# rdspring1/lightning-thunder

Hardware: AMD Instinct MI355X
Metric: tokens/sec/GPU Llama-2-7B pretrain (LitGPT) + speedup vs eager at 1/2/4/8 MI355X (higher is better)
Workload: dtype bf16; 1 GPU; model=Llama-2-7b-hf, global_batch=1, micro_batch=1, seq_len=4096, parallelism=single, mode=thunder, optimizer=AdamW

## Files before the change

lightning_thunder_amd/ops/csrc/attention_bwd.hip:

```cpp
#include "attention.h"

using namespace lta;
using namespace lta::attn;

namespace {

constexpr int kThreads = 256;
typedef __attribute__((address_space(3))) void lds_void;
typedef float f32x4v __attribute__((ext_vector_type(4)));

template <int D> struct BCfg {
  static constexpr int BN = D > 128 ? 32 : 64;
  static constexpr int NKT = BN / 32;
  static constexpr int RSTR = D + 8;
  static constexpr int TSTR = D + 32;
  static constexpr int CH = D / 8;
  static constexpr int KS = D / 16;
  static constexpr int DT = D / 32;
};

struct RowStrides {
  int64_t b, h, t;
};

// ... 126 lines not shown
  using C = BCfg<D>;
  using F = typename Frag<T>::type;
  constexpr int BUF = 2 * kQT * C::RSTR + 2 * kQT * C::TSTR;
  __shared__ __attribute__((aligned(16))) short smem[2 * BUF];
  __shared__ float s_lse[2][kQT], s_delta[2][kQT];
  __shared__ __attribute__((aligned(16))) unsigned s_qterm[2][DROP ? kQT : 4];

  const int n_kb = (Sk + kKB - 1) / kKB;
  (void)n_kb;
  const int kb = (int)blockIdx.y;
  const int nsplit = SPLIT ? ex.hsplit : 1;
  const int bh = SPLIT ? (int)blockIdx.x / nsplit : (int)blockIdx.x;
  const int hs = SPLIT ? (int)blockIdx.x - bh * nsplit : 0;
  const int b = bh / Hkv, hk = bh % Hkv;
  const int group = Hq / Hkv;
  const int gsz = group / nsplit;
  const int hbase = hk * group + hs * gsz;
  const int tid = threadIdx.x, lane = tid & 63;
  const int wave = __builtin_amdgcn_readfirstlane(tid >> 6);
  const int r = lane & 31, h = lane >> 5, g = lane >> 4, l16 = lane & 15;
  const int kw = kb * kKB + wave * 32;
  const int key = kw + r;
  const T* Kb = K + b * ex.sx.kb + hk * ex.sx.kh;
  const T* Vb = V + b * ex.sx.vb + hk * ex.sx.vh;

  F kf[C::KS], vf[C::KS];
  {
    const int krow = min(key, Sk - 1);
#pragma unroll
    for (int s = 0; s < C::KS; ++s) {
      kf[s] = load_frag<F>(Kb + (int64_t)krow * ex.sx.kt + 16 * s + 8 * h);
      vf[s] = load_frag<F>(Vb + (int64_t)krow * ex.sx.vt + 16 * s + 8 * h);
    }
  }
  f32x16 dkacc[C::DT], dvacc[C::DT];
#pragma unroll
  for (int dt = 0; dt < C::DT; ++dt)
#pragma unroll
    for (int i = 0; i < 16; ++i) {
      dkacc[dt][i] = 0.f;
      dvacc[dt][i] = 0.f;
    }

  const int n_qt = (Tq + kQT - 1) / kQT;
  const int qt_begin = CAUSAL ? min((kb * kKB) / kQT, n_qt) : 0;
  const int nq = n_qt - qt_begin;
  const int total = gsz * nq;
  constexpr int NCH = kQT * C::CH, LOADS = (NCH + kThreads - 1) / kThreads;

  uint4 pq[LOADS], po[LOADS];
  float plse = 0.f, pdel = 0.f;
  auto issue = [&](int it) {
    const int hq = hbase + it / nq;
    const int qbase = (qt_begin + it % nq) * kQT;
    const T* Qb = Q + b * ex.sx.qb + hq * ex.sx.qh;
    const T* dOb = dO + b * sdo.b + hq * sdo.h;
#pragma unroll
    for (int c = 0; c < LOADS; ++c) {
      const int id = c * kThreads + tid;
      if (NCH % kThreads != 0 && id >= NCH) break;
      const int row = id / C::CH, ch = id % C::CH;
      const int qc = min(qbase + row, Tq - 1);
      pq[c] = *reinterpret_cast<const uint4*>(Qb + (int64_t)qc * ex.sx.qt + ch * 8);
      po[c] = *reinterpret_cast<const uint4*>(dOb + qc * sdo.t + ch * 8);
    }
    if (tid < kQT) {
      const int qc = min(qbase + tid, Tq - 1);
      plse = LSE[((int64_t)b * Hq + hq) * Tq + qc];
      pdel = DELTA[((int64_t)b * Hq + hq) * Tq + qc];
    }
  };
  auto stash = [&](int it, int buf) {
    const int qbase = (qt_begin + it % nq) * kQT;
    short* Qr = smem + buf * BUF;
    short* dOr = Qr + kQT * C::RSTR;
    short* Qt = dOr + kQT * C::RSTR;
    short* dOt = Qt + kQT * C::TSTR;
#pragma unroll
    for (int c = 0; c < LOADS; ++c) {
      const int id = c * kThreads + tid;
      if (NCH % kThreads != 0 && id >= NCH) break;
      const int row = id / C::CH, ch = id % C::CH;
      uint4 xq = pq[c], xo = po[c];
      if (qbase + row >= Tq) {
        xq = make_uint4(0, 0, 0, 0);
        xo = make_uint4(0, 0, 0, 0);
      }
      *reinterpret_cast<uint4*>(Qr + row * C::RSTR + ch * 8) = xq;
      *reinterpret_cast<uint4*>(dOr + row * C::RSTR + ch * 8) = xo;
      *reinterpret_cast<uint4*>(Qt + row * C::TSTR + ch * 8) = xq;
      *reinterpret_cast<uint4*>(dOt + row * C::TSTR + ch * 8) = xo;
    }
    if (tid < kQT) {
      const bool ok = qbase + tid < Tq && !(MASK && plse == -INFINITY);
      s_lse[buf][tid] = ok ? plse * 1.44269504088896340736f : INFINITY;
      s_delta[buf][tid] = ok ? pdel : 0.f;
      if constexpr (DROP) s_qterm[buf][tid] = rng_q(rng_head(ex, b * Hq + hbase + it / nq), qbase + tid);
    }
  };

  if (total > 0) {
    issue(0);
    stash(0, 0);
  }
  __syncthreads();
  for (int it = 0; it < total; ++it) {
    const int buf = it & 1;
    const bool more = it + 1 < total;
    if (more) issue(it + 1);
    const int qbase = (qt_begin + it % nq) * kQT;
    const short* Qr = smem + buf * BUF;
    const short* dOr = Qr + kQT * C::RSTR;
    const __attribute__((address_space(3))) short* Qt3 =
        (const __attribute__((address_space(3))) short*)(dOr + kQT * C::RSTR);
    const __attribute__((address_space(3))) short* dOt3 = Qt3 + kQT * C::TSTR;
    const float* sl = s_lse[buf];
    const float* sd = s_delta[buf];

    f32x16 sacc, pacc;
#pragma unroll
    for (int i = 0; i < 16; ++i) {
      sacc[i] = 0.f;
      pacc[i] = 0.f;
    }
#pragma unroll
    for (int s = 0; s < C::KS; ++s) {
      const F qa = load_frag<F>(Qr + r * C::RSTR + 16 * s + 8 * h);
      const F oa = load_frag<F>(dOr + r * C::RSTR + 16 * s + 8 * h);
      sacc = mfma(qa, kf[s], sacc);
      pacc = mfma(oa, vf[s], pacc);
    }
    [[maybe_unused]] const int hq_it = hbase + it / nq;
    [[maybe_unused]] unsigned kterm = 0;
    if constexpr (DROP) kterm = rng_k(key);
#pragma unroll
    for (int i = 0; i < 16; ++i) {
      const int qr = acc_row(i, h);
      const int qq = qbase + qr;
      float sv = sacc[i] * scale_log2;
      if constexpr (MASK)
        sv += ex.mask[b * ex.mb + hq_it * ex.mh + (int64_t)min(qq, Tq - 1) * ex.mq + min(key, Sk - 1)] *
              1.44269504088896340736f;
      float p = __builtin_amdgcn_exp2f(sv - sl[qr]);
      p = (key >= Sk || qq >= Tq || (CAUSAL && key > qq)) ? 0.f : p;
      float dp = pacc[i];
      float pd = p;
      if constexpr (DROP) {
        const uint4 qv = rng_tab4(s_qterm[buf], i >> 2, h);
        const unsigned qw4[4] = {qv.x, qv.y, qv.z, qv.w};
        const bool keep = rng_keep(ex, qw4[i & 3], kterm);
        pd = keep ? p * ex.keep_scale : 0.f;
        dp = keep ? dp * ex.keep_scale : 0.f;
      }
      sacc[i] = pd;
      pacc[i] = p * (dp - sd[qr]);
      if constexpr (MGRAD) {
        if (key < Sk && qq < Tq) ex.dmask[(((int64_t)b * Hq + hq_it) * Tq + qq) * Sk + key] = pacc[i];
      }
    }
    F pf0, pf1, df0, df1;
    pack_frag(pf0, sacc, 0);
    pack_frag(pf1, sacc, 1);
    pack_frag(df0, pacc, 0);
    pack_frag(df1, pacc, 1);
#pragma unroll
    for (int dt = 0; dt < C::DT; ++dt) {
      const int col0 = dt * 32 + 16 * (g & 1);
      const F oa0 = tr_frag<F>(dOt3, 4 * h, col0, C::TSTR, l16);
      const F oa1 = tr_frag<F>(dOt3, 16 + 4 * h, col0, C::TSTR, l16);
      const F qa0 = tr_frag<F>(Qt3, 4 * h, col0, C::TSTR, l16);
      const F qa1 = tr_frag<F>(Qt3, 16 + 4 * h, col0, C::TSTR, l16);
      if constexpr (D > 128) {
        mfma_acc_agpr(dvacc[dt], oa0, pf0);
        mfma_acc_agpr(dvacc[dt], oa1, pf1);
        mfma_acc_agpr(dkacc[dt], qa0, df0);
        mfma_acc_agpr(dkacc[dt], qa1, df1);
      } else {
        dvacc[dt] = mfma(oa0, pf0, dvacc[dt]);
        dvacc[dt] = mfma(oa1, pf1, dvacc[dt]);
        dkacc[dt] = mfma(qa0, df0, dkacc[dt]);
        dkacc[dt] = mfma(qa1, df1, dkacc[dt]);
      }
    }
    if (more) stash(it + 1, buf ^ 1);
    __syncthreads();
  }

  if constexpr (D > 128) {
#pragma unroll
    for (int dt = 0; dt < C::DT; ++dt) asm volatile("s_nop 15\n\ts_nop 15" : "+a"(dkacc[dt]), "+a"(dvacc[dt]));
  }
  if (SPLIT && key < Sk) {
    const int nbh = (int)gridDim.x / nsplit;
    float* prow = ex.part + (((int64_t)hs * nbh + bh) * Sk + key) * (2 * D);
#pragma unroll
    for (int dt = 0; dt < C::DT; ++dt)
#pragma unroll
      for (int a = 0; a < 4; ++a) {
        const int d = dt * 32 + 8 * a + 4 * h;
        *reinterpret_cast<float4*>(prow + d) = make_float4(dkacc[dt][4 * a] * scale, dkacc[dt][4 * a + 1] * scale,
                                                           dkacc[dt][4 * a + 2] * scale, dkacc[dt][4 * a + 3] * scale);
        *reinterpret_cast<float4*>(prow + D + d) =
            make_float4(dvacc[dt][4 * a], dvacc[dt][4 * a + 1], dvacc[dt][4 * a + 2], dvacc[dt][4 * a + 3]);
      }
  } else if (key < Sk) {
    T* dkrow = dK + (int64_t)b * ex.sx.dkb + (int64_t)hk * ex.sx.dkh + (int64_t)key * ex.sx.dkt;
    T* dvrow = dV + (int64_t)b * ex.sx.dvb + (int64_t)hk * ex.sx.dvh + (int64_t)key * ex.sx.dvt;
#pragma unroll
    for (int dt = 0; dt < C::DT; ++dt) {
#pragma unroll
      for (int a = 0; a < 4; ++a) {
        const int d = dt * 32 + 8 * a + 4 * h;
        union {
          T v[4];
          uint2 u;
        } pk, pv;
#pragma unroll
        for (int e = 0; e < 4; ++e) {
          pk.v[e] = from_f32<T>(dkacc[dt][4 * a + e] * scale);
          pv.v[e] = from_f32<T>(dvacc[dt][4 * a + e]);
        }
        *reinterpret_cast<uint2*>(dkrow + d) = pk.u;
        *reinterpret_cast<uint2*>(dvrow + d) = pv.u;
      }
    }
  }
}

__device__ __forceinline__ int du_off(int row, int ch) {
  return 2048 * (row >> 3) + 512 * (ch >> 2) + 64 * (row & 7) + 16 * ((ch & 3) ^ ((row >> 2) & 3));
}

__device__ __forceinline__ void tr_frags8(bf16x8 (&f)[8], unsigned ba, unsigned bb) {
  typedef short s16x4v __attribute__((ext_vector_type(4)));
  s16x4v x[16];
  asm volatile(
      "ds_read_b64_tr_b16 %0, %16\n\tds_read_b64_tr_b16 %1, %17\n\t"
      "ds_read_b64_tr_b16 %2, %16 offset:4096\n\tds_read_b64_tr_b16 %3, %17 offset:4096\n\t"
      "ds_read_b64_tr_b16 %4, %16 offset:512\n\tds_read_b64_tr_b16 %5, %17 offset:512\n\t"
      "ds_read_b64_tr_b16 %6, %16 offset:4608\n\tds_read_b64_tr_b16 %7, %17 offset:4608\n\t"
      "ds_read_b64_tr_b16 %8, %16 offset:1024\n\tds_read_b64_tr_b16 %9, %17 offset:1024\n\t"
      "ds_read_b64_tr_b16 %10, %16 offset:5120\n\tds_read_b64_tr_b16 %11, %17 offset:5120\n\t"
      "ds_read_b64_tr_b16 %12, %16 offset:1536\n\tds_read_b64_tr_b16 %13, %17 offset:1536\n\t"
      "ds_read_b64_tr_b16 %14, %16 offset:5632\n\tds_read_b64_tr_b16 %15, %17 offset:5632\n\t"
      "s_waitcnt lgkmcnt(0)"
      : "=&v"(x[0]), "=&v"(x[1]), "=&v"(x[2]), "=&v"(x[3]), "=&v"(x[4]), "=&v"(x[5]), "=&v"(x[6]), "=&v"(x[7]),
        "=&v"(x[8]), "=&v"(x[9]), "=&v"(x[10]), "=&v"(x[11]), "=&v"(x[12]), "=&v"(x[13]), "=&v"(x[14]), "=&v"(x[15])
      : "v"(ba), "v"(bb)
      : "memory");
#pragma unroll
  for (int i = 0; i < 8; ++i) {
    union {
      struct { s16x4v a, b; } s;
      bf16x8 f;
    } u;
    u.s.a = x[2 * i];
    u.s.b = x[2 * i + 1];
    f[i] = u.f;
  }
}
__device__ __forceinline__ void tr_frags8(f16x8 (&f)[8], unsigned ba, unsigned bb) {
  bf16x8 t[8];
  tr_frags8(t, ba, bb);
#pragma unroll
  for (int i = 0; i < 8; ++i) f[i] = __builtin_bit_cast(f16x8, t[i]);
}

typedef short s16x4t __attribute__((ext_vector_type(4)));
__device__ __forceinline__ void tr_issue16(s16x4t (&x)[16], unsigned ba, unsigned bb) {
  asm volatile(
      "ds_read_b64_tr_b16 %0, %16\n\tds_read_b64_tr_b16 %1, %17\n\t"
      "ds_read_b64_tr_b16 %2, %16 offset:4096\n\tds_read_b64_tr_b16 %3, %17 offset:4096\n\t"
      "ds_read_b64_tr_b16 %4, %16 offset:512\n\tds_read_b64_tr_b16 %5, %17 offset:512\n\t"
      "ds_read_b64_tr_b16 %6, %16 offset:4608\n\tds_read_b64_tr_b16 %7, %17 offset:4608\n\t"
      "ds_read_b64_tr_b16 %8, %16 offset:1024\n\tds_read_b64_tr_b16 %9, %17 offset:1024\n\t"
      "ds_read_b64_tr_b16 %10, %16 offset:5120\n\tds_read_b64_tr_b16 %11, %17 offset:5120\n\t"
      "ds_read_b64_tr_b16 %12, %16 offset:1536\n\tds_read_b64_tr_b16 %13, %17 offset:1536\n\t"
      "ds_read_b64_tr_b16 %14, %16 offset:5632\n\tds_read_b64_tr_b16 %15, %17 offset:5632"
      : "=&v"(x[0]), "=&v"(x[1]), "=&v"(x[2]), "=&v"(x[3]), "=&v"(x[4]), "=&v"(x[5]), "=&v"(x[6]), "=&v"(x[7]),
        "=&v"(x[8]), "=&v"(x[9]), "=&v"(x[10]), "=&v"(x[11]), "=&v"(x[12]), "=&v"(x[13]), "=&v"(x[14]), "=&v"(x[15])
      : "v"(ba), "v"(bb)
      : "memory");
}
template <typename F>
__device__ __forceinline__ void tr_wait16(F (&f)[8], s16x4t (&x)[16]) {
  asm volatile("s_waitcnt lgkmcnt(0)"
               : "+v"(x[0]), "+v"(x[1]), "+v"(x[2]), "+v"(x[3]), "+v"(x[4]), "+v"(x[5]), "+v"(x[6]), "+v"(x[7]),
                 "+v"(x[8]), "+v"(x[9]), "+v"(x[10]), "+v"(x[11]), "+v"(x[12]), "+v"(x[13]), "+v"(x[14]), "+v"(x[15])
               :
               : "memory");
#pragma unroll
  for (int i = 0; i < 8; ++i) {
    union {
      struct { s16x4t a, b; } s;
      F f;
    } u;
    u.s.a = x[2 * i];
    u.s.b = x[2 * i + 1];
    f[i] = u.f;
  }
}

typedef int dsi32x4 __attribute__((ext_vector_type(4)));

constexpr int kKB3 = 256;

template <typename T, bool CAUSAL, int STAMP = 0, bool WDS = false, bool SPLIT = false>
__global__ __launch_bounds__(kThreads, 1) void attn_bwd_dkdv_v4_kernel(const T* __restrict__ Q, const T* __restrict__ K,
                                                                       const T* __restrict__ V, const T* __restrict__ dO,
                                                                       const float* __restrict__ LSE,
                                                                       const float* __restrict__ DELTA, T* __restrict__ dK,
                                                                       T* __restrict__ dV, int Hq, int Hkv, int Tq, int Sk,
                                                                       float scale, float scale_log2, RowStrides sdo, QKVStrides sx,
                                                                       int qrev = 0, uint64_t* dbg = nullptr,
                                                                       T* __restrict__ dSt = nullptr, int hsplit = 1,
                                                                       float* __restrict__ part = nullptr) {
  constexpr int D = 128;
  using C = BCfg<D>;
  using F = typename Frag<T>::type;
  constexpr int NST = 3;
  constexpr int IMG = kQT * 256;
  constexpr int STAGE = 2 * IMG + 256;
  constexpr int VOFF = NST * STAGE;
  constexpr int SBASE = VOFF + kKB3 * C::RSTR * 2;
  __shared__ __attribute__((aligned(1024))) char smem[SBASE + (STAMP ? 4 * 64 * 8 * 8 : 0)];
  short* Vs = reinterpret_cast<short*>(smem + VOFF);

  const int kb = (int)blockIdx.y;
  const int nsplit = SPLIT ? hsplit : 1;
  const int bh = SPLIT ? (int)blockIdx.x / nsplit : (int)blockIdx.x, hs = SPLIT ? (int)blockIdx.x % nsplit : 0;
  const int b = bh / Hkv, hk = bh % Hkv;
  const int group = Hq / Hkv;
  const int gsz = group / nsplit, hbase = hk * group + hs * gsz;
  const int tid = threadIdx.x, lane = tid & 63;
  const int wave = __builtin_amdgcn_readfirstlane(tid >> 6);
  const int r = lane & 31, h = lane >> 5;
  const int kw = kb * kKB3 + wave * 64;
  const T* Kb = K + b * sx.kb + hk * sx.kh;
  const T* Vb = V + b * sx.vb + hk * sx.vh;

#pragma unroll
  for (int c = 0; c < kKB3 * C::CH / kThreads; ++c) {
    const int id = c * kThreads + tid;
    const int row = id / C::CH, ch = id % C::CH;
    const int vr = min(kb * kKB3 + row, Sk - 1);
    *reinterpret_cast<uint4*>(Vs + row * C::RSTR + ch * 8) = *reinterpret_cast<const uint4*>(Vb + (int64_t)vr * sx.vt + ch * 8);
  }
  F kf[2][C::KS];
#pragma unroll
  for (int j = 0; j < 2; ++j) {
    const int kr = min(kw + 32 * j + r, Sk - 1);
#pragma unroll
    for (int s = 0; s < C::KS; ++s) kf[j][s] = load_frag<F>(Kb + (int64_t)kr * sx.kt + 16 * s + 8 * h);
  }

  f32x16 dkacc[2][C::DT], dvacc[2][C::DT];
#pragma unroll
  for (int j = 0; j < 2; ++j)
#pragma unroll
    for (int dt = 0; dt < C::DT; ++dt)
#pragma unroll
      for (int i = 0; i < 16; ++i) {
        dkacc[j][dt][i] = 0.f;
        dvacc[j][dt][i] = 0.f;
      }

  const int n_qt = (Tq + kQT - 1) / kQT;
  const int qt_begin = CAUSAL ? min((kb * kKB3) / kQT, n_qt) : 0;
  const int nq = n_qt - qt_begin;
  const int total = gsz * nq;

  float plse = 0.f, pdel = 0.f;
  auto stash_stats = [&](int st) {
    if (wave == 0 && lane < kQT) {
      float* sp = reinterpret_cast<float*>(smem + st * STAGE + 2 * IMG);
      sp[lane] = -plse * 1.44269504088896340736f;
      sp[kQT + lane] = pdel;
    }
  };
  auto issue = [&](int hi, int ti, int st) {
    const int hq = hbase + hi;
    const int qbase = (qt_begin + (qrev ? nq - 1 - ti : ti)) * kQT;
    const T* Qb = Q + b * sx.qb + hq * sx.qh;
    const T* dOb = dO + b * sdo.b + hq * sdo.h;
    char* qimg = smem + st * STAGE;
    if (wave == 0) {
      const int64_t srow = ((int64_t)b * Hq + hq) * Tq + min(qbase + (lane & 31), Tq - 1);
      asm volatile("global_load_dword %0, %2, off\n\tglobal_load_dword %1, %3, off"
                   : "=&v"(plse), "=&v"(pdel)
                   : "v"(LSE + srow), "v"(DELTA + srow)
                   : "memory");
    }
#pragma unroll
    for (int i = 0; i < 2; ++i) {
      const int k = wave * 2 + i;
      const int u = 64 * k + lane;
      const int row = ((u >> 7) << 3) | ((u >> 2) & 7);
      const int ch = (((u >> 5) & 3) << 2) | ((u & 3) ^ ((row >> 2) & 3));
      const int qc = min(qbase + row, Tq - 1);
      __builtin_amdgcn_global_load_lds((const void*)(Qb + (int64_t)qc * sx.qt + ch * 8),
                                       (lds_void*)(qimg + k * 1024), 16, 0, 0);
      __builtin_amdgcn_global_load_lds((const void*)(dOb + qc * sdo.t + ch * 8),
                                       (lds_void*)(qimg + IMG + k * 1024), 16, 0, 0);
    }
  };
  auto wait_all_but_newest = [&](bool after_stores) {
    if (WDS && after_stores)
      asm volatile("s_waitcnt vmcnt(8)" : "+v"(plse), "+v"(pdel)::"memory");
    else
      asm volatile("s_waitcnt vmcnt(4)" : "+v"(plse), "+v"(pdel)::"memory");
  };

  int nhi = 0, nti = 0;
  auto advance = [&]() {
    if (++nti == nq) {
      nti = 0;
      ++nhi;
    }
  };
  asm volatile("s_waitcnt vmcnt(0)" ::: "memory");
  if (total > 0) {
    issue(nhi, nti, 0);
    advance();
    asm volatile("s_waitcnt vmcnt(0)" : "+v"(plse), "+v"(pdel)::"memory");
    stash_stats(0);
  }
  if (total > 1) {
    issue(nhi, nti, 1);
    advance();
    wait_all_but_newest(false);
    stash_stats(1);
  }
  __syncthreads();

  unsigned tr_a, tr_b;
  {
    const int l16 = lane & 15, g = lane >> 4;
    const int q = l16 >> 2, p = l16 & 3, cl = 2 * (g & 1) + (p >> 1);
    const unsigned base = (unsigned)(uintptr_t)(__attribute__((address_space(3))) char*)smem;
    tr_a = base + 64 * (4 * h + q) + 16 * (cl ^ h) + 8 * (p & 1);
    tr_b = base + 2048 + 64 * (4 * h + q) + 16 * (cl ^ (2 + h)) + 8 * (p & 1);
  }
  constexpr float kLog2e = 1.44269504088896340736f;
  int ti = 0, st = 0;
  auto stamp = [&](int it, int k) {
    if constexpr (STAMP != 0) {
      if (blockIdx.x == 0 && blockIdx.y == 0 && it < 64) {
        __builtin_amdgcn_sched_barrier(0);
        const uint64_t ts = __builtin_amdgcn_s_memtime();
        if (lane == 0) *reinterpret_cast<uint64_t*>(smem + SBASE + ((wave * 64 + it) * 8 + k) * 8) = ts;
        __builtin_amdgcn_sched_barrier(0);
      }
    }
  };
  for (int it = 0; it < total; ++it) {
    stamp(it, 0);
    const bool issue_next = it + 2 < total;
    const int st2 = st >= 1 ? st - 1 : 2;
    if (issue_next) issue(nhi, nti, st2);
    const int qt_abs = qt_begin + (qrev ? nq - 1 - ti : ti);
    const int qbase = qt_abs * kQT;
    {
      const char* qimg = smem + st * STAGE;
      const char* oimg = qimg + IMG;
      const float* sl = reinterpret_cast<const float*>(qimg + 2 * IMG);
      f32x4v L[4], Dl[4];
#pragma unroll
      for (int a = 0; a < 4; ++a) L[a] = *reinterpret_cast<const f32x4v*>(sl + 4 * h + 8 * a);
      f32x16 sacc[2], pacc[2];
      F pf[2][2], df[2][2];
#pragma unroll
      for (int j = 0; j < 2; ++j)
#pragma unroll
        for (int i = 0; i < 16; ++i) {
          sacc[j][i] = 0.f;
          pacc[j][i] = 0.f;
        }
      {
        F qa[C::KS];
#pragma unroll
        for (int s = 0; s < C::KS; ++s) qa[s] = load_frag<F>(qimg + du_off(r, 2 * s + h));
#pragma unroll
        for (int s = 0; s < C::KS; ++s)
#pragma unroll
          for (int j = 0; j < 2; ++j) sacc[j] = mfma(qa[s], kf[j][s], sacc[j]);
      }
      __builtin_amdgcn_sched_barrier(0);
      stamp(it, 1);
      {
        F oa = load_frag<F>(oimg + du_off(r, h));
        F va0 = load_frag<F>(Vs + (wave * 64 + r) * C::RSTR + 8 * h);
        F va1 = load_frag<F>(Vs + (wave * 64 + 32 + r) * C::RSTR + 8 * h);
#pragma unroll
        for (int s = 0; s < C::KS; ++s) {
          F ob = oa, vb0 = va0, vb1 = va1;
          if (s + 1 < C::KS) {
            ob = load_frag<F>(oimg + du_off(r, 2 * (s + 1) + h));
            vb0 = load_frag<F>(Vs + (wave * 64 + r) * C::RSTR + 16 * (s + 1) + 8 * h);
            vb1 = load_frag<F>(Vs + (wave * 64 + 32 + r) * C::RSTR + 16 * (s + 1) + 8 * h);
          }
          pacc[0] = mfma(oa, va0, pacc[0]);
          pacc[1] = mfma(oa, va1, pacc[1]);
          const int j = s >> 2, i0 = 4 * (s & 3);
#pragma unroll
          for (int i = i0; i < i0 + 4; ++i)
            sacc[j][i] = __builtin_amdgcn_exp2f(__builtin_fmaf(sacc[j][i], scale_log2, L[i >> 2][i & 3]));
          if (s == 4 || s == 5) pack_frag(pf[0][s - 4], sacc[0], s - 4);
          __builtin_amdgcn_sched_barrier(0);
          oa = ob;
          va0 = vb0;
          va1 = vb1;
        }
      }
      stamp(it, 2);
#pragma unroll
      for (int a = 0; a < 4; ++a) Dl[a] = *reinterpret_cast<const f32x4v*>(sl + kQT + 4 * h + 8 * a);
      s16x4t xr[16];
      tr_issue16(xr, tr_a + (unsigned)(st * STAGE + IMG), tr_b + (unsigned)(st * STAGE + IMG));
#pragma unroll
      for (int j = 0; j < 2; ++j) {
        const int key = kw + 32 * j + r;
        const bool masked = (CAUSAL && kw + 32 * j + 31 > qbase) || kw + 32 * j + 32 > Sk || qbase + kQT > Tq;
        if (masked) {
#pragma unroll
          for (int i = 0; i < 16; ++i) {
            const int qq = qbase + acc_row(i, h);
            if (key >= Sk || qq >= Tq || (CAUSAL && key > qq)) sacc[j][i] = 0.f;
          }
          if (j == 0) {
            pack_frag(pf[0][0], sacc[0], 0);
            pack_frag(pf[0][1], sacc[0], 1);
          }
        }
      }
      pack_frag(pf[1][0], sacc[1], 0);
      pack_frag(pf[1][1], sacc[1], 1);
      stamp(it, 3);
      {
        F xt[8];
        tr_wait16(xt, xr);
#pragma unroll
        for (int dt = 0; dt < C::DT; ++dt) {
#pragma unroll
          for (int j = 0; j < 2; ++j) {
            mfma_acc_agpr(dvacc[j][dt], xt[2 * dt], pf[j][0]);
            mfma_acc_agpr(dvacc[j][dt], xt[2 * dt + 1], pf[j][1]);
            const int jj = dt >> 1, i0 = 8 * (dt & 1) + 4 * j;
#pragma unroll
            for (int i = i0; i < i0 + 4; ++i) pacc[jj][i] = sacc[jj][i] * (pacc[jj][i] - Dl[i >> 2][i & 3]);
            asm volatile("" : "+v"(pacc[jj]));
            __builtin_amdgcn_sched_barrier(0);
          }
          if (dt & 1) {
            pack_frag(df[dt >> 1][0], pacc[dt >> 1], 0);
            pack_frag(df[dt >> 1][1], pacc[dt >> 1], 1);
            if (dt == 1) tr_issue16(xr, tr_a + (unsigned)(st * STAGE), tr_b + (unsigned)(st * STAGE));
            __builtin_amdgcn_sched_barrier(0);
          }
        }
        stamp(it, 4);
        tr_wait16(xt, xr);
#pragma unroll
        for (int dt = 0; dt < C::DT; ++dt)
#pragma unroll
          for (int j = 0; j < 2; ++j) {
            mfma_acc_agpr(dkacc[j][dt], xt[2 * dt], df[j][0]);
            mfma_acc_agpr(dkacc[j][dt], xt[2 * dt + 1], df[j][1]);
          }
        if constexpr (WDS) {
          const int hq_cur = hbase + it / nq;
          const int nqb = (Tq + 255) >> 8;
          const uint64_t wa = (uint64_t)(uintptr_t)(dSt + ((((int64_t)(b * Hq + hq_cur) * nqb + (qbase >> 8)) * Sk + kw) * 256 +
                                                           (qbase & 255)));
          const uint64_t wu = ((uint64_t)(uint32_t)__builtin_amdgcn_readfirstlane((int)(wa >> 32)) << 32) |
                              (uint32_t)__builtin_amdgcn_readfirstlane((int)(uint32_t)wa);
          const int wbytes = __builtin_amdgcn_readfirstlane(max(0, min(64, Sk - kw)) * 512);
          const __amdgpu_buffer_rsrc_t rs =
              __builtin_amdgcn_make_buffer_rsrc((void*)(uintptr_t)wu, (short)0, wbytes, 0x00020000);
          const int loff = (r * 256 + 8 * h) * 2;
#pragma unroll
          for (int j = 0; j < 2; ++j) {
            __builtin_amdgcn_raw_buffer_store_b128(__builtin_bit_cast(dsi32x4, df[j][0]), rs, loff, j * 16384, 2);
            __builtin_amdgcn_raw_buffer_store_b128(__builtin_bit_cast(dsi32x4, df[j][1]), rs, loff, j * 16384 + 32, 2);
          }
        }
      }
    }
    stamp(it, 5);
    if (issue_next) {
      advance();
      wait_all_but_newest(true);
      stash_stats(st2);
    } else {
      asm volatile("s_waitcnt vmcnt(0)" ::: "memory");
    }
    stamp(it, 6);
    asm volatile("s_waitcnt lgkmcnt(0)" ::: "memory");
    __builtin_amdgcn_s_barrier();
    asm volatile("" ::: "memory");
    stamp(it, 7);
    ti = ti + 1 == nq ? 0 : ti + 1;
    st = st == 2 ? 0 : st + 1;
  }
  if constexpr (STAMP != 0) {
    if (blockIdx.x == 0 && blockIdx.y == 0 && dbg != nullptr) {
      __syncthreads();
      for (int i = tid; i < 4 * 64 * 8; i += kThreads) dbg[i] = *reinterpret_cast<const uint64_t*>(smem + SBASE + i * 8);
    }
  }
#pragma unroll
  for (int j = 0; j < 2; ++j)
#pragma unroll
    for (int dt = 0; dt < C::DT; ++dt) asm volatile("s_nop 15\n\ts_nop 15" : "+a"(dkacc[j][dt]), "+a"(dvacc[j][dt]));

  if constexpr (SPLIT) {
#pragma unroll
    for (int j = 0; j < 2; ++j) {
      const int key = kw + 32 * j + r;
      if (key < Sk) {
        const int64_t nbh = gridDim.x / nsplit;
        float* prow = part + (((int64_t)hs * nbh + bh) * Sk + key) * 256;
        const bool rope = sx.rope_cos != nullptr;
        store_row_d128_f32(prow, dkacc[j], scale, h, rope ? sx.rope_cos + (int64_t)key * 128 : nullptr,
                           rope ? sx.rope_sin + (int64_t)key * 128 : nullptr);
        store_row_d128_f32(prow + 128, dvacc[j], 1.f, h, nullptr, nullptr);
      }
    }
    return;
  }
#pragma unroll
  for (int j = 0; j < 2; ++j) {
    const int key = kw + 32 * j + r;
    if (key < Sk) {
      T* dkrow = dK + (int64_t)b * sx.dkb + (int64_t)hk * sx.dkh + (int64_t)key * sx.dkt;
      T* dvrow = dV + (int64_t)b * sx.dvb + (int64_t)hk * sx.dvh + (int64_t)key * sx.dvt;
      const bool rope = sx.rope_cos != nullptr;
      store_row_d128(dkrow, dkacc[j], scale, h, rope ? sx.rope_cos + (int64_t)key * 128 : nullptr,
                     rope ? sx.rope_sin + (int64_t)key * 128 : nullptr);
      store_row_d128(dvrow, dvacc[j], 1.f, h, nullptr, nullptr);
    }
  }
}

constexpr int kBM = 128;
constexpr int kBN = 64;

template <typename T, int D, bool CAUSAL, int EX = 0>
__global__ __launch_bounds__(kThreads, (EX || D > 128) ? 1 : 2) void attn_bwd_dq_kernel(const T* __restrict__ Q, const T* __restrict__ K,
                                                                  const T* __restrict__ V, const T* __restrict__ dO,
                                                                  const float* __restrict__ LSE,
                                                                  const float* __restrict__ DELTA, T* __restrict__ dQ,
                                                                  int Hq, int Hkv, int Tq, int Sk, float scale,
                                                                  float scale_log2, RowStrides sdo, AttnExtra ex) {
  constexpr bool MASK = EX & kExMask, DROP = EX & kExDrop;
  using C = BCfg<D>;
  using F = typename Frag<T>::type;
  __shared__ __attribute__((aligned(16))) short smem[2 * C::BN * C::RSTR + C::BN * C::TSTR];
  __shared__ __attribute__((aligned(16))) unsigned ktab[DROP ? 4 * C::BN : 4];
  short* Kr = smem;
  short* Vr = Kr + C::BN * C::RSTR;
  short* Kt = Vr + C::BN * C::RSTR;
  const __attribute__((address_space(3))) short* Kt3 = (const __attribute__((address_space(3))) short*)Kt;

  const int n_qt = (Tq + kBM - 1) / kBM;
  const int qt = n_qt - 1 - (int)blockIdx.y;
  const int bh = blockIdx.x;
  const int b = bh / Hq, hq = bh % Hq;
  const int hk = hq / (Hq / Hkv);
  const T* Qb = Q + b * ex.sx.qb + hq * ex.sx.qh;
  const T* dOb = dO + b * sdo.b + hq * sdo.h;
  const T* Kb = K + b * ex.sx.kb + hk * ex.sx.kh;
  const T* Vb = V + b * ex.sx.vb + hk * ex.sx.vh;

  const int tid = threadIdx.x, lane = tid & 63;
  const int wave = __builtin_amdgcn_readfirstlane(tid >> 6);
  const int r = lane & 31, h = lane >> 5, g = lane >> 4, l16 = lane & 15;
  const int q0 = qt * kBM + wave * 32;
  const int qi = q0 + r;
  const int qrow = min(qi, Tq - 1);

  F qf[C::KS], of[C::KS];
#pragma unroll
  for (int s = 0; s < C::KS; ++s) {
    qf[s] = load_frag<F>(Qb + (int64_t)qrow * ex.sx.qt + 16 * s + 8 * h);
    of[s] = load_frag<F>(dOb + qrow * sdo.t + 16 * s + 8 * h);
  }
  float lse2 = LSE[((int64_t)b * Hq + hq) * Tq + qrow] * 1.44269504088896340736f;
  if constexpr (MASK) lse2 = (lse2 == -INFINITY) ? INFINITY : lse2;
  const float dlt = DELTA[((int64_t)b * Hq + hq) * Tq + qrow];
  const float* mrow = nullptr;
  if constexpr (MASK) mrow = ex.mask + b * ex.mb + hq * ex.mh + (int64_t)qrow * ex.mq;
  unsigned qterm = 0;
  if constexpr (DROP) qterm = rng_q(rng_head(ex, bh), qi);

  f32x16 dqacc[C::DT];
#pragma unroll
  for (int dt = 0; dt < C::DT; ++dt)
#pragma unroll
    for (int i = 0; i < 16; ++i) dqacc[dt][i] = 0.f;

  int n_tiles = (Sk + C::BN - 1) / C::BN;
  if (CAUSAL) n_tiles = min(n_tiles, (min(qt * kBM + kBM, Tq) + C::BN - 1) / C::BN);
  constexpr int LOADS = C::BN * C::CH / kThreads;
  static_assert(C::BN * C::CH % kThreads == 0, "K/V staging must cover the tile");

  uint4 pk[LOADS], pv[LOADS];
  auto issue = [&](int t) {
#pragma unroll
    for (int c = 0; c < LOADS; ++c) {
      const int id = c * kThreads + tid;
      const int row = id / C::CH, ch = id % C::CH;
      const int kc = min(t * C::BN + row, Sk - 1);
      pk[c] = *reinterpret_cast<const uint4*>(Kb + (int64_t)kc * ex.sx.kt + ch * 8);
      pv[c] = *reinterpret_cast<const uint4*>(Vb + (int64_t)kc * ex.sx.vt + ch * 8);
    }
  };
  if (n_tiles > 0) issue(0);
  for (int t = 0; t < n_tiles; ++t) {
    __syncthreads();
#pragma unroll
    for (int c = 0; c < LOADS; ++c) {
      const int id = c * kThreads + tid;
      const int row = id / C::CH, ch = id % C::CH;
      uint4 xk = pk[c], xv = pv[c];
      if (t * C::BN + row >= Sk) {
        xk = make_uint4(0, 0, 0, 0);
        xv = make_uint4(0, 0, 0, 0);
      }
      *reinterpret_cast<uint4*>(Kr + row * C::RSTR + ch * 8) = xk;
      *reinterpret_cast<uint4*>(Vr + row * C::RSTR + ch * 8) = xv;
      *reinterpret_cast<uint4*>(Kt + row * C::TSTR + ch * 8) = xk;
    }
    __syncthreads();
    if (t + 1 < n_tiles) issue(t + 1);

    f32x16 sacc[C::NKT], pacc[C::NKT];
#pragma unroll
    for (int kt = 0; kt < C::NKT; ++kt)
#pragma unroll
      for (int i = 0; i < 16; ++i) {
        sacc[kt][i] = 0.f;
        pacc[kt][i] = 0.f;
      }
#pragma unroll
    for (int s = 0; s < C::KS; ++s) {
#pragma unroll
      for (int kt = 0; kt < C::NKT; ++kt) {
        const F ka = load_frag<F>(Kr + (kt * 32 + r) * C::RSTR + 16 * s + 8 * h);
        const F va = load_frag<F>(Vr + (kt * 32 + r) * C::RSTR + 16 * s + 8 * h);
        sacc[kt] = mfma(ka, qf[s], sacc[kt]);
        pacc[kt] = mfma(va, of[s], pacc[kt]);
      }
    }
    const int kbase = t * C::BN;
    [[maybe_unused]] unsigned* krow = ktab + wave * C::BN;
    if constexpr (DROP)
      if (lane < C::BN) krow[lane] = rng_k(kbase + lane);
    if constexpr (MASK) {
#pragma unroll
      for (int kt = 0; kt < C::NKT; ++kt)
#pragma unroll
        for (int j = 0; j < 4; ++j) {
          const float4 mv = *reinterpret_cast<const float4*>(mrow + kbase + kt * 32 + 8 * j + 4 * h);
          sacc[kt][4 * j + 0] = sacc[kt][4 * j + 0] * scale_log2 + mv.x * 1.44269504088896340736f;
          sacc[kt][4 * j + 1] = sacc[kt][4 * j + 1] * scale_log2 + mv.y * 1.44269504088896340736f;
          sacc[kt][4 * j + 2] = sacc[kt][4 * j + 2] * scale_log2 + mv.z * 1.44269504088896340736f;
          sacc[kt][4 * j + 3] = sacc[kt][4 * j + 3] * scale_log2 + mv.w * 1.44269504088896340736f;
        }
    }
#pragma unroll
    for (int kt = 0; kt < C::NKT; ++kt) {
#pragma unroll
      for (int i = 0; i < 16; ++i) {
        const int kk = kbase + kt * 32 + acc_row(i, h);
        float p = __builtin_amdgcn_exp2f((MASK ? sacc[kt][i] : sacc[kt][i] * scale_log2) - lse2);
        p = (kk >= Sk || (CAUSAL && kk > qi)) ? 0.f : p;
        float dp = pacc[kt][i];
        if constexpr (DROP) {
          const uint4 kv = rng_tab4(krow + kt * 32, i >> 2, h);
          const unsigned kw4[4] = {kv.x, kv.y, kv.z, kv.w};
          const bool keep = rng_keep(ex, qterm, kw4[i & 3]);
          dp = keep ? dp * ex.keep_scale : 0.f;
        }
        pacc[kt][i] = p * (dp - dlt);
      }
    }
    F df[C::NKT][2];
#pragma unroll
    for (int kt = 0; kt < C::NKT; ++kt) {
      pack_frag(df[kt][0], pacc[kt], 0);
      pack_frag(df[kt][1], pacc[kt], 1);
    }
#pragma unroll
    for (int dt = 0; dt < C::DT; ++dt) {
      const int col0 = dt * 32 + 16 * (g & 1);
#pragma unroll
      for (int kt = 0; kt < C::NKT; ++kt) {
#pragma unroll
        for (int s = 0; s < 2; ++s) {
          const F ka = tr_frag<F>(Kt3, kt * 32 + 16 * s + 4 * h, col0, C::TSTR, l16);
          dqacc[dt] = mfma(ka, df[kt][s], dqacc[dt]);
        }
      }
    }
  }

  if (qi < Tq) {
    T* drow = dQ + (int64_t)b * ex.sx.dqb + (int64_t)hq * ex.sx.dqh + (int64_t)qi * ex.sx.dqt;
#pragma unroll
    for (int dt = 0; dt < C::DT; ++dt) {
#pragma unroll
      for (int a = 0; a < 4; ++a) {
        const int d = dt * 32 + 8 * a + 4 * h;
        union {
          T v[4];
          uint2 u;
        } pk;
#pragma unroll
        for (int e = 0; e < 4; ++e) pk.v[e] = from_f32<T>(dqacc[dt][4 * a + e] * scale);
        *reinterpret_cast<uint2*>(drow + d) = pk.u;
      }
    }
  }
}

constexpr int kQB3 = 256;
constexpr int kKT3 = 32;

template <typename T, bool CAUSAL>
__global__ __launch_bounds__(kThreads, 1) void attn_bwd_dq_v4_kernel(const T* __restrict__ Q, const T* __restrict__ K,
                                                                     const T* __restrict__ V, const T* __restrict__ dO,
                                                                     const float* __restrict__ LSE,
                                                                     const float* __restrict__ DELTA, T* __restrict__ dQ,
                                                                     int Hq, int Hkv, int Tq, int Sk, float scale,
                                                                     float scale_log2, RowStrides sdo, QKVStrides sx,
                                                                     const T* __restrict__ O = nullptr, RowStrides so = {}) {
  constexpr int D = 128;
  using C = BCfg<D>;
  using F = typename Frag<T>::type;
  constexpr int NST = 3;
  constexpr int IMG = kKT3 * 256;
  constexpr int STAGE = 2 * IMG;
  constexpr int OOFF = NST * STAGE;
  __shared__ __attribute__((aligned(1024))) char smem[OOFF + kQB3 * C::RSTR * 2];
  short* Os = reinterpret_cast<short*>(smem + OOFF);

  const int n_qb = (Tq + kQB3 - 1) / kQB3;
  const int qb = n_qb - 1 - (int)blockIdx.y;
  const int bh = blockIdx.x;
  const int b = bh / Hq, hq = bh % Hq;
  const int hk = hq / (Hq / Hkv);
  const int tid = threadIdx.x, lane = tid & 63;
  const int wave = __builtin_amdgcn_readfirstlane(tid >> 6);
  const int r = lane & 31, h = lane >> 5;
  const int qw = qb * kQB3 + wave * 64;
  const T* Qb = Q + b * sx.qb + hq * sx.qh;
  const T* dOb = dO + b * sdo.b + hq * sdo.h;
  const T* Kb = K + b * sx.kb + hk * sx.kh;
  const T* Vb = V + b * sx.vb + hk * sx.vh;

#pragma unroll
  for (int c = 0; c < kQB3 * C::CH / kThreads; ++c) {
    const int id = c * kThreads + tid;
    const int row = id / C::CH, ch = id % C::CH;
    const int orow = min(qb * kQB3 + row, Tq - 1);
    *reinterpret_cast<uint4*>(Os + row * C::RSTR + ch * 8) = *reinterpret_cast<const uint4*>(dOb + (int64_t)orow * sdo.t + ch * 8);
  }
  constexpr float kLog2e = 1.44269504088896340736f;
  F qf[2][C::KS];
  float nl2[2], dl[2];
#pragma unroll
  for (int j = 0; j < 2; ++j) {
    const int qr = min(qw + 32 * j + r, Tq - 1);
#pragma unroll
    for (int s = 0; s < C::KS; ++s) qf[j][s] = load_frag<F>(Qb + (int64_t)qr * sx.qt + 16 * s + 8 * h);
    nl2[j] = -LSE[((int64_t)b * Hq + hq) * Tq + qr] * kLog2e;
    if (O != nullptr) {
      const T* Orow = O + (int64_t)b * so.b + (int64_t)hq * so.h + (int64_t)qr * so.t;
      const T* Drow = dOb + (int64_t)qr * sdo.t;
      float acc = 0.f;
#pragma unroll
      for (int s = 0; s < C::KS; ++s) {
        const F ov = load_frag<F>(Orow + 16 * s + 8 * h), dv = load_frag<F>(Drow + 16 * s + 8 * h);
#pragma unroll
        for (int e = 0; e < 8; ++e) acc += (float)dv[e] * (float)ov[e];
      }
      dl[j] = acc + __shfl_xor(acc, 32, 64);
      if (h == 0 && qw + 32 * j + r < Tq) const_cast<float*>(DELTA)[((int64_t)b * Hq + hq) * Tq + qw + 32 * j + r] = dl[j];
    } else {
      dl[j] = DELTA[((int64_t)b * Hq + hq) * Tq + qr];
    }
  }

  f32x16 dqacc[2][C::DT];
#pragma unroll
  for (int j = 0; j < 2; ++j)
#pragma unroll
    for (int dt = 0; dt < C::DT; ++dt)
#pragma unroll
      for (int i = 0; i < 16; ++i) dqacc[j][dt][i] = 0.f;

  int n_kt = (Sk + kKT3 - 1) / kKT3;
  if (CAUSAL) n_kt = min(n_kt, (min(qb * kQB3 + kQB3, Tq) + kKT3 - 1) / kKT3);

// ... 665 lines not shown
```

Measured before the change: 24630 tokens/s.

## Use buffer-load DMA with precomputed offsets and software-pipeline LDS fragment reads in dKdV

Replaces per-iteration global_load_lds address computation with buffer_load...lds using precomputed per-lane offsets and scalar base pointers that advance incrementally per tile and head. It also rewrites the Q·K and dO·V MFMA loops to issue ds_read_b128 fragment loads ahead of use, in a three-deep rotation with explicit lgkmcnt waits. The goal is to cut VALU address arithmetic and hide LDS latency behind MFMAs. It adds register pressure and relies on hand-counted waitcnt values, which would cause hazards if miscounted.

```diff
diff --git a/lightning_thunder_amd/ops/csrc/attention_bwd.hip b/lightning_thunder_amd/ops/csrc/attention_bwd.hip
--- a/lightning_thunder_amd/ops/csrc/attention_bwd.hip
+++ b/lightning_thunder_amd/ops/csrc/attention_bwd.hip
@@ -452,6 +452,28 @@
 }
 
 typedef int dsi32x4 __attribute__((ext_vector_type(4)));
+
+__device__ __forceinline__ dsi32x4 make_rsrc(uint64_t base, uint32_t bytes) {
+  return dsi32x4{(int)(uint32_t)base, (int)((uint32_t)(base >> 32) & 0xffffu), (int)bytes, 0x00020000};
+}
+__device__ __forceinline__ void dma16(uint32_t dst, int voff, dsi32x4 rsrc) {
+  asm volatile("s_mov_b32 m0, %0\n\ts_nop 0\n\tbuffer_load_dwordx4 %1, %2, 0 offen lds"
+               :
+               : "s"(dst), "v"(voff), "s"(rsrc)
+               : "memory", "m0");
+}
+
+__device__ __forceinline__ void frag_issue(dsi32x4& x, unsigned addr, int off) {
+  asm volatile("ds_read_b128 %0, %1 offset:%2" : "=&v"(x) : "v"(addr), "i"(off) : "memory");
+}
+__device__ __forceinline__ void frag_wait(dsi32x4& x, int n) {
+  asm volatile("s_waitcnt lgkmcnt(%1)" : "+v"(x) : "i"(n) : "memory");
+  __builtin_amdgcn_sched_barrier(0);
+}
+__device__ __forceinline__ void frag_wait(dsi32x4& x, dsi32x4& y, dsi32x4& z, int n) {
+  asm volatile("s_waitcnt lgkmcnt(%3)" : "+v"(x), "+v"(y), "+v"(z) : "i"(n) : "memory");
+  __builtin_amdgcn_sched_barrier(0);
+}
 
 constexpr int kKB3 = 256;
 
@@ -528,30 +550,46 @@
       sp[kQT + lane] = pdel;
     }
   };
-  auto issue = [&](int hi, int ti, int st) {
+  const uint32_t lds0 = (uint32_t)(uintptr_t)(__attribute__((address_space(3))) char*)smem;
+  const uint32_t qrow_b = (uint32_t)sx.qt * (uint32_t)sizeof(T), orow_b = (uint32_t)sdo.t * (uint32_t)sizeof(T);
+  int vq[2], vo[2];
+#pragma unroll
+  for (int i = 0; i < 2; ++i) {
+    const int u = 64 * (wave * 2 + i) + lane;
+    const int row = ((u >> 7) << 3) | ((u >> 2) & 7);
+    const int ch = (((u >> 5) & 3) << 2) | ((u & 3) ^ ((row >> 2) & 3));
+    vq[i] = row * (int)qrow_b + ch * 16;
+    vo[i] = row * (int)orow_b + ch * 16;
+  }
+  const int stat_l = (lane & 31) * 4;
+  const int tstep = qrev ? -kQT : kQT;
+  const int64_t qstep = (int64_t)tstep * (int64_t)qrow_b, ostep = (int64_t)tstep * (int64_t)orow_b;
+  uint64_t nqa = 0, noa = 0, nlse = 0, ndel = 0;
+  int nqb = 0;
+  auto enter_head = [&](int hi) {
     const int hq = hbase + hi;
-    const int qbase = (qt_begin + (qrev ? nq - 1 - ti : ti)) * kQT;
-    const T* Qb = Q + b * sx.qb + hq * sx.qh;
-    const T* dOb = dO + b * sdo.b + hq * sdo.h;
-    char* qimg = smem + st * STAGE;
+    nqb = (qt_begin + (qrev ? nq - 1 : 0)) * kQT;
+    nqa = (uint64_t)(uintptr_t)(Q + b * sx.qb + hq * sx.qh + (int64_t)nqb * sx.qt);
+    noa = (uint64_t)(uintptr_t)(dO + b * sdo.b + hq * sdo.h + (int64_t)nqb * sdo.t);
+    const int64_t srow = ((int64_t)b * Hq + hq) * Tq;
+    nlse = (uint64_t)(uintptr_t)(LSE + srow);
+    ndel = (uint64_t)(uintptr_t)(DELTA + srow);
+  };
+  auto issue = [&](int st) {
     if (wave == 0) {
-      const int64_t srow = ((int64_t)b * Hq + hq) * Tq + min(qbase + (lane & 31), Tq - 1);
-      asm volatile("global_load_dword %0, %2, off\n\tglobal_load_dword %1, %3, off"
+      const int soff = min(nqb * 4 + stat_l, (Tq - 1) * 4);
+      asm volatile("global_load_dword %0, %2, %3\n\tglobal_load_dword %1, %2, %4"
                    : "=&v"(plse), "=&v"(pdel)
-                   : "v"(LSE + srow), "v"(DELTA + srow)
+                   : "v"(soff), "s"(nlse), "s"(ndel)
                    : "memory");
     }
+    const uint32_t last = (uint32_t)(min(kQT, Tq - nqb) - 1);
+    const dsi32x4 rq = make_rsrc(nqa, last * qrow_b + 256u), ro = make_rsrc(noa, last * orow_b + 256u);
+    const uint32_t qimg = lds0 + (uint32_t)(st * STAGE + wave * 2048);
 #pragma unroll
     for (int i = 0; i < 2; ++i) {
-      const int k = wave * 2 + i;
-      const int u = 64 * k + lane;
-      const int row = ((u >> 7) << 3) | ((u >> 2) & 7);
-      const int ch = (((u >> 5) & 3) << 2) | ((u & 3) ^ ((row >> 2) & 3));
-      const int qc = min(qbase + row, Tq - 1);
-      __builtin_amdgcn_global_load_lds((const void*)(Qb + (int64_t)qc * sx.qt + ch * 8),
-                                       (lds_void*)(qimg + k * 1024), 16, 0, 0);
-      __builtin_amdgcn_global_load_lds((const void*)(dOb + qc * sdo.t + ch * 8),
-                                       (lds_void*)(qimg + IMG + k * 1024), 16, 0, 0);
+      dma16(qimg + i * 1024, vq[i], rq);
+      dma16(qimg + IMG + i * 1024, vo[i], ro);
     }
   };
   auto wait_all_but_newest = [&](bool after_stores) {
@@ -565,18 +603,27 @@
   auto advance = [&]() {
     if (++nti == nq) {
       nti = 0;
-      ++nhi;
+      if (++nhi < gsz) enter_head(nhi);
+    } else {
+      nqa += qstep;
+      noa += ostep;
+      nqb += tstep;
     }
   };
   asm volatile("s_waitcnt vmcnt(0)" ::: "memory");
+#pragma unroll
+  for (int j = 0; j < 2; ++j)
+#pragma unroll
+    for (int s = 0; s < C::KS; ++s) asm volatile("" : "+v"(kf[j][s]));
   if (total > 0) {
-    issue(nhi, nti, 0);
+    enter_head(0);
+    issue(0);
     advance();
     asm volatile("s_waitcnt vmcnt(0)" : "+v"(plse), "+v"(pdel)::"memory");
     stash_stats(0);
   }
   if (total > 1) {
-    issue(nhi, nti, 1);
+    issue(1);
     advance();
     wait_all_but_newest(false);
     stash_stats(1);
@@ -587,12 +634,15 @@
   {
     const int l16 = lane & 15, g = lane >> 4;
     const int q = l16 >> 2, p = l16 & 3, cl = 2 * (g & 1) + (p >> 1);
-    const unsigned base = (unsigned)(uintptr_t)(__attribute__((address_space(3))) char*)smem;
-    tr_a = base + 64 * (4 * h + q) + 16 * (cl ^ h) + 8 * (p & 1);
-    tr_b = base + 2048 + 64 * (4 * h + q) + 16 * (cl ^ (2 + h)) + 8 * (p & 1);
-  }
+    tr_a = lds0 + 64 * (4 * h + q) + 16 * (cl ^ h) + 8 * (p & 1);
+    tr_b = lds0 + 2048 + 64 * (4 * h + q) + 16 * (cl ^ (2 + h)) + 8 * (p & 1);
+  }
+  const unsigned fr[2] = {lds0 + (unsigned)du_off(r, h), lds0 + (unsigned)du_off(r, 2 + h)};
+  const unsigned fv = lds0 + (unsigned)(VOFF + ((wave * 64 + r) * C::RSTR + 8 * h) * 2);
+  constexpr int VH1 = 32 * C::RSTR * 2;
+  const unsigned fl = lds0 + (unsigned)(2 * IMG + 16 * h);
   constexpr float kLog2e = 1.44269504088896340736f;
-  int ti = 0, st = 0;
+  int ti = 0, st = 0, hcur = hbase;
   auto stamp = [&](int it, int k) {
     if constexpr (STAMP != 0) {
       if (blockIdx.x == 0 && blockIdx.y == 0 && it < 64) {
@@ -607,16 +657,19 @@
     stamp(it, 0);
     const bool issue_next = it + 2 < total;
     const int st2 = st >= 1 ? st - 1 : 2;
-    if (issue_next) issue(nhi, nti, st2);
     const int qt_abs = qt_begin + (qrev ? nq - 1 - ti : ti);
     const int qbase = qt_abs * kQT;
     {
-      const char* qimg = smem + st * STAGE;
-      const char* oimg = qimg + IMG;
-      const float* sl = reinterpret_cast<const float*>(qimg + 2 * IMG);
+      const unsigned so = (unsigned)(st * STAGE);
+      const unsigned qa[2] = {fr[0] + so, fr[1] + so};
+      const float* sl = reinterpret_cast<const float*>(smem + st * STAGE + 2 * IMG);
+      dsi32x4 lx[4], qx[C::KS], bx[3][3];
       f32x4v L[4], Dl[4];
 #pragma unroll
-      for (int a = 0; a < 4; ++a) L[a] = *reinterpret_cast<const f32x4v*>(sl + 4 * h + 8 * a);
+      for (int a = 0; a < 4; ++a) frag_issue(lx[a], fl + so, 32 * a);
+#pragma unroll
+      for (int s = 0; s < C::KS; ++s) frag_issue(qx[s], qa[s & 1], 512 * (s >> 1));
+      if (issue_next) issue(st2);
       f32x16 sacc[2], pacc[2];
       F pf[2][2], df[2][2];
 #pragma unroll
@@ -626,41 +679,45 @@
           sacc[j][i] = 0.f;
           pacc[j][i] = 0.f;
         }
-      {
-        F qa[C::KS];
-#pragma unroll
-        for (int s = 0; s < C::KS; ++s) qa[s] = load_frag<F>(qimg + du_off(r, 2 * s + h));
-#pragma unroll
-        for (int s = 0; s < C::KS; ++s)
-#pragma unroll
-          for (int j = 0; j < 2; ++j) sacc[j] = mfma(qa[s], kf[j][s], sacc[j]);
+#pragma unroll
+      for (int s = 0; s < C::KS; ++s) {
+        if (s == 4 || s == 6) {
+          const int sb = (s - 4) >> 1;
+          frag_issue(bx[sb][0], qa[sb & 1], IMG);
+          frag_issue(bx[sb][1], fv, 32 * sb);
+          frag_issue(bx[sb][2], fv, VH1 + 32 * sb);
+        }
+        frag_wait(qx[s], C::KS - 1 - s + (s >= 6 ? 6 : s >= 4 ? 3 : 0));
+        if (s == 0) {
+          asm volatile("" : "+v"(lx[0]), "+v"(lx[1]), "+v"(lx[2]), "+v"(lx[3]));
+#pragma unroll
+          for (int a = 0; a < 4; ++a) L[a] = __builtin_bit_cast(f32x4v, lx[a]);
+        }
+        const F q = __builtin_bit_cast(F, qx[s]);
+#pragma unroll
+        for (int j = 0; j < 2; ++j) sacc[j] = mfma(q, kf[j][s], sacc[j]);
       }
       __builtin_amdgcn_sched_barrier(0);
       stamp(it, 1);
-      {
-        F oa = load_frag<F>(oimg + du_off(r, h));
-        F va0 = load_frag<F>(Vs + (wave * 64 + r) * C::RSTR + 8 * h);
-        F va1 = load_frag<F>(Vs + (wave * 64 + 32 + r) * C::RSTR + 8 * h);
-#pragma unroll
-        for (int s = 0; s < C::KS; ++s) {
-          F ob = oa, vb0 = va0, vb1 = va1;
-          if (s + 1 < C::KS) {
-            ob = load_frag<F>(oimg + du_off(r, 2 * (s + 1) + h));
-            vb0 = load_frag<F>(Vs + (wave * 64 + r) * C::RSTR + 16 * (s + 1) + 8 * h);
-            vb1 = load_frag<F>(Vs + (wave * 64 + 32 + r) * C::RSTR + 16 * (s + 1) + 8 * h);
-          }
-          pacc[0] = mfma(oa, va0, pacc[0]);
-          pacc[1] = mfma(oa, va1, pacc[1]);
-          const int j = s >> 2, i0 = 4 * (s & 3);
-#pragma unroll
-          for (int i = i0; i < i0 + 4; ++i)
-            sacc[j][i] = __builtin_amdgcn_exp2f(__builtin_fmaf(sacc[j][i], scale_log2, L[i >> 2][i & 3]));
-          if (s == 4 || s == 5) pack_frag(pf[0][s - 4], sacc[0], s - 4);
-          __builtin_amdgcn_sched_barrier(0);
-          oa = ob;
-          va0 = vb0;
-          va1 = vb1;
+#pragma unroll
+      for (int s = 0; s < C::KS; ++s) {
+        if (s + 2 < C::KS) {
+          const int sb = s + 2;
+          frag_issue(bx[sb % 3][0], qa[sb & 1], IMG + 512 * (sb >> 1));
+          frag_issue(bx[sb % 3][1], fv, 32 * sb);
+          frag_issue(bx[sb % 3][2], fv, VH1 + 32 * sb);
         }
+        frag_wait(bx[s % 3][0], bx[s % 3][1], bx[s % 3][2], 3 * min(2, C::KS - 1 - s));
+        const F oa = __builtin_bit_cast(F, bx[s % 3][0]);
+        pacc[0] = mfma(oa, __builtin_bit_cast(F, bx[s % 3][1]), pacc[0]);
+        pacc[1] = mfma(oa, __builtin_bit_cast(F, bx[s % 3][2]), pacc[1]);
+        __builtin_amdgcn_sched_barrier(0);
+        const int j = s >> 2, i0 = 4 * (s & 3);
+#pragma unroll
+        for (int i = i0; i < i0 + 4; ++i)
+          sacc[j][i] = __builtin_amdgcn_exp2f(__builtin_fmaf(sacc[j][i], scale_log2, L[i >> 2][i & 3]));
+        if (s == 4 || s == 5) pack_frag(pf[0][s - 4], sacc[0], s - 4);
+        __builtin_amdgcn_sched_barrier(0);
       }
       stamp(it, 2);
 #pragma unroll
@@ -718,9 +775,8 @@
             mfma_acc_agpr(dkacc[j][dt], xt[2 * dt + 1], df[j][1]);
           }
         if constexpr (WDS) {
-          const int hq_cur = hbase + it / nq;
-          const int nqb = (Tq + 255) >> 8;
-          const uint64_t wa = (uint64_t)(uintptr_t)(dSt + ((((int64_t)(b * Hq + hq_cur) * nqb + (qbase >> 8)) * Sk + kw) * 256 +
+          const int nqb8 = (Tq + 255) >> 8;
+          const uint64_t wa = (uint64_t)(uintptr_t)(dSt + ((((int64_t)(b * Hq + hcur) * nqb8 + (qbase >> 8)) * Sk + kw) * 256 +
                                                            (qbase & 255)));
           const uint64_t wu = ((uint64_t)(uint32_t)__builtin_amdgcn_readfirstlane((int)(wa >> 32)) << 32) |
                               (uint32_t)__builtin_amdgcn_readfirstlane((int)(uint32_t)wa);
@@ -749,7 +805,10 @@
     __builtin_amdgcn_s_barrier();
     asm volatile("" ::: "memory");
     stamp(it, 7);
-    ti = ti + 1 == nq ? 0 : ti + 1;
+    if (++ti == nq) {
+      ti = 0;
+      ++hcur;
+    }
     st = st == 2 ? 0 : st + 1;
   }
   if constexpr (STAMP != 0) {
```

Result: no change. 24680 tokens/s (median of 6 runs) (+0.2%).
